# westlake-repl/PixelRec

Hardware: AMD Instinct MI355X
Metric: user-sequences/sec at emb=512 seq_len=50 (SASRec IDNet training step: fwd+bwd+AdamW) (higher is better)
Workload: dtype f32; 1 GPU; BASELINE.json configs[1]: SASRec IDNet emb=512 seq_len=50, 400001 items, 4 heads, inner 2x, 2 layers, BPR loss vs 1 sampled negative, dropout 0.1, AdamW lr 1e-4 wd 0.1; batch_per_gpu=64, global_batch=64, seq_len=50, n_items=400001, embedding_size=512, parallelism=dp1, hip_graph=True

## Files before the change

### include/pxr.h

```cpp
#ifndef PXR_H_
#define PXR_H_
#include <stdint.h>

#ifdef __cplusplus
extern "C" {
#endif

#define PXR_OK 0
#define PXR_ERR_BAD_ARG (-1)
#define PXR_ERR_LAUNCH (-2)
#define PXR_ERR_WORKSPACE (-3)

#define PXR_ABI_VERSION 302
int pxr_version(void);
const char* pxr_last_error(void);
const char* pxr_target_arch(void);

int pxr_dropout_keep_host(uint64_t seed, uint32_t stream_id, uint64_t first_index, int64_t n, float p,
                          uint8_t* keep_out);

int pxr_set_status_word(int32_t* dev_word);

int pxr_embed_gather_f32(const float* table, int64_t N, int D, const int64_t* idx, int64_t n, float* out,
                         void* stream);
// ... 101 lines not shown
                          const int* dy_exp, const int* const* dy_exp_dev, const void* const* x, const int64_t* x_plane_stride,
                          const int64_t* x_panel_rows, const int* x_exp, const int* const* x_exp_dev, float* const* dW,
                          float* const* db, const int* T, const int* N, const int* K, int tile_hint, void* stream);
int pxr_h2_split_auto_multi_f32(int n, const float* const* x, const int64_t* rows, const int64_t* cols, const int64_t* ldx,
                                void* const* planes, const int64_t* plane_stride, const int64_t* panel_rows, int col_stats,
                                float* stats, int* exps, void* stream);
int pxr_h2_bound_exp(const float* a_max, const float* b_colsum, float factor, int* exp_out, void* stream);
int pxr_ln_bwd_stat_f32(const float* dy, const float* xhat, const float* rstd, const float* gamma, int rows, int D, float* dz,
                        float* dx, float* dgamma, float* dbeta, float p_drop, uint64_t seed, uint32_t stream_id,
                        const int64_t* step_dev, void* ws, int64_t ws_bytes, float* stat, float* zero, int zero_n, void* stream);
int pxr_ln_bwd_res_f32(const float* dy, const float* xhat, const float* rstd, const float* gamma, const float* res, int rows, int D,
                       float* dz, float* dgamma, float* dbeta, void* ws, int64_t ws_bytes, float* stat, void* stream);
int pxr_h2_split_parts_f32(const float* x, int64_t rows, int64_t cols, int64_t ldx, void* planes, int64_t plane_stride,
                           int64_t panel_rows, const float* parts, int n_parts, float* stats, int* exps,
                           const float* bound_b_colsum, float bound_factor, int* bound_exp_out, void* stream);
int pxr_attn_bwd_stat_f32(const float* dctx, int64_t ld_ctx, const float* q, const float* k, const float* v, int64_t ld,
                          const float* probs, int B, int H, int L, int d, float* dq, float* dk, float* dv, int64_t ld_d,
                          float p_drop, uint64_t seed, uint32_t stream_id, const int64_t* step_dev, float* stat, void* stream);
int pxr_ln_bwd_h2s_f32(const float* pos_score, const float* neg_score, const float* table, int64_t n_table, const int64_t* items,
                       const int64_t* masked_index, int B, int L, float grad_scale, const float* grad_scale_dev, float* coef,
                       const float* dy, const float* xhat, const float* rstd, const float* gamma, int rows, int D, float* dz,
                       float* dgamma, float* dbeta, float p_drop, uint64_t seed, uint32_t stream_id, const int64_t* step_dev,
                       void* ws, int64_t ws_bytes, void* g_planes, int64_t g_plane_stride, int64_t g_panel_rows,
                       const int* g_exp_dev, float* stat, float* zero, int zero_n, int64_t id_bstride, int64_t pos_off,
                       int64_t neg_off, void* stream);
int pxr_attn_bwd_h2s_f32(const float* dctx, int64_t ld_ctx, const float* q, const float* k, const float* v, int64_t ld,
                         const float* probs, int B, int H, int L, int d, float p_drop, uint64_t seed, uint32_t stream_id,
                         const int64_t* step_dev, void* g_planes, int64_t g_plane_stride, int64_t g_panel_rows, int g_cols,
                         int col_q, int col_k, int col_v, const int* g_exp_dev, float* stat, void* stream);
int pxr_h2_sites_update(int n, const float* const* parts, const int* n_parts, const int* rows, const float* const* bound_b,
                        float bound_factor, int headroom, float decay, float* run_max, int* exps, float* stats, int* bexp, void* stream);

int pxr_attn_planes_supported(int L, int d);
int pxr_score_topk_clock_out(uint64_t* clk2);
int pxr_gemm_reset_flags(void);
int pxr_grouped_dw_planes_f32(int n, const void* const* dy, const int64_t* dy_plane_stride, const int64_t* dy_panel_rows,
                              const void* const* x, const int64_t* x_plane_stride, const int64_t* x_panel_rows,
                              float* const* dW, float* const* db, const int* T, const int* N, const int* K, int tile_hint,
                              void* stream);

int pxr_tower_attn_supported(int T, int d);
int pxr_tower_attn_fwd_f32(const float* q, const float* k, const float* v, int64_t ld, int64_t images, int heads, int T, int d,
                           float scale, float* ctx, int64_t ld_ctx, void* ctx_planes, int64_t ctx_plane_stride,
                           int64_t ctx_panel_rows, int planes_fmt, float* lse, void* stream);
int pxr_tower_attn_bwd_f32(const float* q, const float* k, const float* v, int64_t ld, const float* dctx, const float* ctx,
                           int64_t ld_c, const float* lse, int64_t images, int heads, int T, int d, float scale, float* dq,
                           float* dk, float* dv, int64_t ld_d, float* delta_ws, void* stream);
int pxr_softmax_rows_f32(float* S, int64_t rows, int T, int ld, float scale, void* stream);
int pxr_softmax_rows_bwd_f32(const float* P, float* dP, int64_t rows, int T, int ld, float scale, void* stream);
int pxr_vit_embed_f32(const float* patches, const float* cls, const float* pos, float* out, int64_t n, int T, int H,
                      void* stream);
int pxr_token_mean_f32(const float* x, float* out, int64_t n, int T, int D, void* stream);
int pxr_token_mean_relu_bwd_f32(const float* dout, const float* act, float* dact, int64_t n, int T, int D, void* stream);
int pxr_attn_rows_fwd_f32(float* S, float* PD, const int64_t* keymask, int64_t km_bstride, int B, int H, int L, int ld,
                          float p_drop, uint64_t seed, uint32_t stream_id, const int64_t* step_dev, int d, int causal,
                          void* stream);
int pxr_attn_rows_bwd_f32(const float* P, float* dPD, int B, int H, int L, int ld, float p_drop, uint64_t seed,
                          uint32_t stream_id, const int64_t* step_dev, int d, void* stream);
int pxr_add_f32(const float* a, const float* b, float* out, int64_t n, void* stream);
int pxr_dropout_f32(const float* x, float* y, int64_t n, float p, uint64_t seed, uint32_t stream_id, const int64_t* step_dev,
                    void* stream);

int pxr_linear_fwd_f32(const float* x, const float* W, const float* b, float* y, float* pre, int M, int N, int K,
                       int act, void* stream);
int pxr_linear_bwd_input_f32(const float* dy, const float* W, float* dx, const float* dgelu_pre, const float* add,
                             const float* mul, int M, int N, int K, void* stream);
// ... 240 lines not shown
```

### pixelrec_amd/csrc/attention.hip

```cpp
#include <stdlib.h>

#include "planes.cuh"

namespace pxr {

constexpr int ATT_MAXL = 64;
constexpr int ATT_DC = 128;
constexpr int ATT_KLD = ATT_DC + 4;

#define PXR_ATTN_STAT_SLOTS 64
struct AttnArgs {
  const float* q; const float* k; const float* v;
  int64_t ld;
  const int64_t* keymask; int64_t km_bstride;
  float* ctx; int64_t ld_ctx;
  float* probs;
  const float* dctx; float* dq; float* dk; float* dv; int64_t ld_d;
  int B, H, L, d;
  float sqrt_d;
  float p_drop; uint32_t drop_thr; uint32_t stream; uint64_t seed;
  const int64_t* step_dev;
  P3Mat op;
  int pcol[3];
  int op_fmt;
  int32_t* status;
  const int* gexp;
  float* stat;
};

__device__ __forceinline__ void stage_tile(float* tile, int tstride, const float* src, int64_t ld, int L, int w) {
  const int q4 = w >> 2;
  for (int f = threadIdx.x; f < L * q4; f += blockDim.x) {
    const int row = f / q4, c = (f - row * q4) * 4;
    *reinterpret_cast<float4*>(tile + row * tstride + c) = *reinterpret_cast<const float4*>(src + (int64_t)row * ld + c);
  }
}

template <int NW>
__device__ __forceinline__ void score_accumulate(float (&acc)[64 / NW], const float* sA, const float* sB, int L, int w,
                                                 int wave, int lane) {
  const float* brow = sB + lane * ATT_KLD;
#pragma unroll
  for (int gg = 0; gg < 16 / NW; ++gg) {
    const int i0 = wave + 4 * NW * gg;
    if (i0 >= L) break;
    float a0 = 0.f, a1 = 0.f, a2 = 0.f, a3 = 0.f;
    const float* r0 = sA + (i0)*ATT_DC;
    const float* r1 = sA + (i0 + NW) * ATT_DC;
    const float* r2 = sA + (i0 + 2 * NW) * ATT_DC;
    const float* r3 = sA + (i0 + 3 * NW) * ATT_DC;
    for (int c = 0; c < w; c += 4) {
      const float4 kb = *reinterpret_cast<const float4*>(brow + c);
      const float4 q0 = *reinterpret_cast<const float4*>(r0 + c);
      const float4 q1 = *reinterpret_cast<const float4*>(r1 + c);
      const float4 q2 = *reinterpret_cast<const float4*>(r2 + c);
      const float4 q3 = *reinterpret_cast<const float4*>(r3 + c);
      a0 += q0.x * kb.x + q0.y * kb.y + q0.z * kb.z + q0.w * kb.w;
      a1 += q1.x * kb.x + q1.y * kb.y + q1.z * kb.z + q1.w * kb.w;
      a2 += q2.x * kb.x + q2.y * kb.y + q2.z * kb.z + q2.w * kb.w;
      a3 += q3.x * kb.x + q3.y * kb.y + q3.z * kb.z + q3.w * kb.w;
// ... 579 lines not shown
    const int i = wave + NW * g;
    if (i < L) sS[i * ATT_SLD + lane] = dsrow[g];
  }
  __syncthreads();
  zero_acc<TN>(acc);
  if (mine) lds_mma<true, false, TN>(acc, sS, ATT_SLD, sK, ATT_KLD, wm * 32, n_base, 64, lane);
  if (a.stat && mine) take();
  if (a.dq) store_acc<TN>(acc, a.dq + dbase, a.ld_d, wm * 32, n_base, L, d, lane);
  if (a.op.p) store_acc_planes<TN, NT>(acc, mine, sV, wm * 32, n_base, L, d, lane, a.op, (int64_t)b * L, a.pcol[0] + h * d, PXR_PLANES_BF16X3, a.status, gsc);
  zero_acc<TN>(acc);
  if (mine) lds_mma<false, false, TN>(acc, sS, ATT_SLD, sQ, ATT_KLD, wm * 32, n_base, 64, lane);
  if (a.stat && mine) take();
  if (a.dk) store_acc<TN>(acc, a.dk + dbase, a.ld_d, wm * 32, n_base, L, d, lane);
  if (a.op.p) store_acc_planes<TN, NT>(acc, mine, sV, wm * 32, n_base, L, d, lane, a.op, (int64_t)b * L, a.pcol[1] + h * d, PXR_PLANES_BF16X3, a.status, gsc);
  if (a.stat) {
    __shared__ float smax[NW];
    gmax = wave_max(gmax);
    if (lane == 0) smax[wave] = gmax;
    __syncthreads();
    if (threadIdx.x == 0) {
      float m = smax[0];
#pragma unroll
      for (int w = 1; w < NW; ++w) m = fmaxf(m, smax[w]);
      float* slot = a.stat + (bh & (PXR_ATTN_STAT_SLOTS - 1));
      if (m > __hip_atomic_load(slot, __ATOMIC_RELAXED, __HIP_MEMORY_SCOPE_AGENT)) atomicMax(reinterpret_cast<int*>(slot), __float_as_int(m));
    }
  }
}

constexpr int ATT2_TR = 52;
constexpr int ATT2_NT = 512;
constexpr int ATT2_NP = (ATT2_TR * (ATT_DC / 4) + ATT2_NT - 1) / ATT2_NT;

__device__ __forceinline__ void tile2_load(float4 (&v)[ATT2_NP], const float* src, int64_t ld, int L, int w) {
  const int q4 = w >> 2;
#pragma unroll
  for (int p = 0; p < ATT2_NP; ++p) {
    const int f = threadIdx.x + p * ATT2_NT;
    const int row = f / q4, c = (f - row * q4) * 4;
    v[p] = make_float4(0.f, 0.f, 0.f, 0.f);
    if (row < L) v[p] = *reinterpret_cast<const float4*>(src + (int64_t)row * ld + c);
  }
}
__device__ __forceinline__ void tile2_store(float* tile, const float4 (&v)[ATT2_NP], int L, int w) {
  const int q4 = w >> 2;
#pragma unroll
  for (int p = 0; p < ATT2_NP; ++p) {
    const int f = threadIdx.x + p * ATT2_NT;
    const int row = f / q4, c = (f - row * q4) * 4;
    if (row <= L) *reinterpret_cast<float4*>(tile + row * ATT_KLD + c) = v[p];
  }
}

template <bool A_KC, bool B_KC, int TN>
__device__ __forceinline__ void lds_mma_z(f32x16 (&acc)[TN], const float* sA, int lda, int za, const float* sB, int ldb, int zb,
                                          int m_base, int n_base, int K, int lane) {
  const int h = lane >> 5, r = lane & 31;
  const int arow = min(m_base + r, za);
  int brow[TN];
#pragma unroll
  for (int j = 0; j < TN; ++j) brow[j] = min(n_base + j * 32 + r, zb);
  for (int k0 = 0; k0 < K; k0 += 8) {
    float a[4], b[TN][4];
    if constexpr (A_KC) {
      const float4 v = *reinterpret_cast<const float4*>(sA + arow * lda + k0 + h * 4);
      a[0] = v.x; a[1] = v.y; a[2] = v.z; a[3] = v.w;
    } else {
#pragma unroll
      for (int t = 0; t < 4; ++t) a[t] = sA[min(k0 + h * 4 + t, za) * lda + m_base + r];
    }
#pragma unroll
    for (int j = 0; j < TN; ++j) {
      if constexpr (B_KC) {
        const float4 v = *reinterpret_cast<const float4*>(sB + brow[j] * ldb + k0 + h * 4);
        b[j][0] = v.x; b[j][1] = v.y; b[j][2] = v.z; b[j][3] = v.w;
      } else {
#pragma unroll
        for (int t = 0; t < 4; ++t) b[j][t] = sB[min(k0 + h * 4 + t, zb) * ldb + n_base + j * 32 + r];
      }
    }
#pragma unroll
    for (int t = 0; t < 4; ++t)
#pragma unroll
      for (int j = 0; j < TN; ++j) acc[j] = __builtin_amdgcn_mfma_f32_32x32x2f32(a[t], b[j][t], acc[j], 0, 0, 0);
  }
}

__device__ __forceinline__ void acc_to_tile2(const f32x16& acc, bool mine, float* tile, int m_base, int n_base, int L, int lane) {
  if (!mine) return;
  const int h = lane >> 5, r = lane & 31;
#pragma unroll
  for (int e = 0; e < 16; ++e) {
    const int row = m_base + (e & 3) + 8 * (e >> 2) + 4 * h;
    if (row < L) tile[row * ATT_KLD + n_base + r] = acc[e];
  }
}
__device__ __forceinline__ void tile2_to_planes(const float* tile, int L, int w, const P3Mat& P, int64_t row0, int col0, int fmt,
                                                int32_t* status, float stale_scale = 0.f) {
  const int cpr = w >> 3;
  for (int q = threadIdx.x; q < L * cpr; q += ATT2_NT) {
    const int row = q / cpr, c8 = (q - row * cpr) * 8;
    const float4 x0 = *reinterpret_cast<const float4*>(tile + row * ATT_KLD + c8);
    const float4 x1 = *reinterpret_cast<const float4*>(tile + row * ATT_KLD + c8 + 4);
    const float v[8] = {x0.x, x0.y, x0.z, x0.w, x1.x, x1.y, x1.z, x1.w};
    if (stale_scale != 0.f) px_store8_h2s(P, status, row0 + row, col0 + c8, v, stale_scale);
    else px_store8(P, fmt, status, row0 + row, col0 + c8, v);
  }
}

template <bool CAUSAL>
__device__ __forceinline__ void attn_fwd_mfma2_body(AttnArgs a) {
  if (a.step_dev) a.seed += (uint64_t)a.step_dev[0];
  constexpr int NW = 8;
  __shared__ __attribute__((aligned(16))) float T0[ATT2_TR * ATT_KLD];
  __shared__ __attribute__((aligned(16))) float T1[ATT2_TR * ATT_KLD];
  __shared__ __attribute__((aligned(16))) float sS[ATT_MAXL * ATT_SLD];
  const int lane = threadIdx.x & 63, wave = threadIdx.x >> 6;
  const int bh = xcd_remap(blockIdx.x, gridDim.x), b = bh / a.H, h = bh - b * a.H;
  const int L = a.L, d = a.d, Kp = (L + 7) & ~7;
  const int64_t base = (int64_t)b * L * a.ld + (int64_t)h * d;
  float4 rq[ATT2_NP], rk[ATT2_NP], rv[ATT2_NP];
  tile2_load(rq, a.q + base, a.ld, L, d);
  tile2_load(rk, a.k + base, a.ld, L, d);
  tile2_load(rv, a.v + base, a.ld, L, d);
  const bool key_real = (lane < L) && (a.keymask[(int64_t)b * a.km_bstride + lane] != 0);
  tile2_store(T0, rq, L, d);
  tile2_store(T1, rk, L, d);
  __syncthreads();
  if (wave < 4) {
    const int wm = wave >> 1, wn = wave & 1;
    f32x16 accS[1];
    zero_acc<1>(accS);
    lds_mma_z<true, true, 1>(accS, T0, ATT_KLD, L, T1, ATT_KLD, L, wm * 32, wn * 32, d, lane);
    const int hh = lane >> 5, r = lane & 31;
// ... 119 lines not shown
  __syncthreads();
#pragma unroll
  for (int g = 0; g < ROWS; ++g) {
    const int i = wave + NW * g;
    if (i < L) sS[i * ATT_SLD + lane] = dsrow[g];
  }
  if (a.op.p) {
    acc_to_tile2(acc[0], mine, T0, wm * 32, n_base, L, lane);
    __syncthreads();
    tile2_to_planes(T0, L, d, a.op, (int64_t)b * L, a.pcol[2] + h * d, PXR_PLANES_BF16X3, a.status, gsc);
    __syncthreads();
  }
  tile2_store(T0, r0, L, d);
  __syncthreads();
  zero_acc<1>(acc);
  zero_acc<1>(acc2);
  if (mine) {
    lds_mma_z<true, false, 1>(acc, sS, ATT_SLD, 63, T1, ATT_KLD, L, wm * 32, n_base, Kp, lane);
    lds_mma_z<false, false, 1>(acc2, sS, ATT_SLD, 63, T0, ATT_KLD, L, wm * 32, n_base, Kp, lane);
  }
  if (a.stat && mine) { take(acc[0]); take(acc2[0]); }
  if (a.dq) store_acc<1>(acc, a.dq + dbase, a.ld_d, wm * 32, n_base, L, d, lane);
  if (a.dk) store_acc<1>(acc2, a.dk + dbase, a.ld_d, wm * 32, n_base, L, d, lane);
  if (a.op.p) {
    __syncthreads();
    acc_to_tile2(acc[0], mine, T1, wm * 32, n_base, L, lane);
    acc_to_tile2(acc2[0], mine, T0, wm * 32, n_base, L, lane);
    __syncthreads();
    tile2_to_planes(T1, L, d, a.op, (int64_t)b * L, a.pcol[0] + h * d, PXR_PLANES_BF16X3, a.status, gsc);
    tile2_to_planes(T0, L, d, a.op, (int64_t)b * L, a.pcol[1] + h * d, PXR_PLANES_BF16X3, a.status, gsc);
  }
  if (a.stat) {
    __shared__ float smax[NW];
    gmax = wave_max(gmax);
    if (lane == 0) smax[wave] = gmax;
    __syncthreads();
    if (threadIdx.x == 0) {
      float m = smax[0];
#pragma unroll
      for (int w = 1; w < NW; ++w) m = fmaxf(m, smax[w]);
      float* slot = a.stat + (bh & (PXR_ATTN_STAT_SLOTS - 1));
      if (m > __hip_atomic_load(slot, __ATOMIC_RELAXED, __HIP_MEMORY_SCOPE_AGENT)) atomicMax(reinterpret_cast<int*>(slot), __float_as_int(m));
    }
  }
}

constexpr int ATTL_MAXL = 128;
constexpr int ATTL_SLD = ATTL_MAXL + 4;
constexpr int ATTL_DC = 64;
constexpr int ATTL_KLD = ATTL_DC + 4;
constexpr int ATTL_NT = 512;

__device__ __forceinline__ void stage_tile_long(float* tile, int tstride, const float* src, int64_t ld, int L, int w) {
  const int q4 = w >> 2;
  const int total = ATTL_MAXL * q4;
  float4 v[4];
#pragma unroll
  for (int p = 0; p < 4; ++p) {
    const int f = threadIdx.x + p * ATTL_NT;
    v[p] = make_float4(0.f, 0.f, 0.f, 0.f);
    if (f < total) {
      const int row = f / q4, c = (f - row * q4) * 4;
      if (row < L) v[p] = *reinterpret_cast<const float4*>(src + (int64_t)row * ld + c);
    }
  }
#pragma unroll
// ... 182 lines not shown
}

using namespace pxr;

static int attn_mfma_waves() {
  static const int nw = getenv("PXR_ATTN_MFMA_WAVES") ? atoi(getenv("PXR_ATTN_MFMA_WAVES")) : 8;
  return nw == 8 ? 8 : 4;
}

static int attn_waves() {
  static int nw = 0;
  if (nw == 0) {
    const char* e = getenv("PXR_ATTN_WAVES");
    const int v = e ? atoi(e) : 8;
    nw = (v == 4 || v == 16) ? v : 8;
  }
  return nw;
}

static bool attn_use_two(int L, int d) {
  const char* e = getenv("PXR_ATTN_TWO");
  return L < ATT2_TR && d <= ATT_DC && attn_mfma_waves() == 8 && !(e && atoi(e) == 0);
}

static bool attn_use_mfma(int d) {
  static int flag = -1;
  if (flag < 0) {
    const char* e = getenv("PXR_ATTN_MFMA");
    flag = (e && atoi(e) == 0) ? 0 : 1;
  }
  return flag == 1 && (d % 8) == 0;
}

static int attn_check(int B, int H, int L, int d, int64_t ld, const char* who) {
  PXR_REQUIRE(B >= 0 && H > 0 && L > 0 && d > 0, "%s: bad shape", who);
  PXR_REQUIRE(L <= ATTL_MAXL, "%s: L=%d > %d positions is not supported", who, L, ATTL_MAXL);
  PXR_REQUIRE(L <= ATT_MAXL || (attn_use_mfma(d)), "%s: L=%d > %d needs the MFMA kernels (head size %d %% 8 == 0)", who, L,
              ATT_MAXL, d);
  PXR_REQUIRE(d % 4 == 0 && ld % 4 == 0, "%s: d and ld must be multiples of 4", who);
  return PXR_OK;
}

extern "C" int pxr_attn_planes_supported(int L, int d) { return (L <= ATT_MAXL && attn_use_mfma(d) && d <= ATT_DC && d % 8 == 0) ? 1 : 0; }

extern "C" int pxr_attn_fwd_f32(const float* q, const float* k, const float* v, int64_t ld, const int64_t* keymask,
                                int64_t km_bstride, int B, int H, int L, int d, float* ctx, int64_t ld_ctx, float* probs,
                                float p_drop, uint64_t seed, uint32_t stream_id, const int64_t* step_dev, void* ctx_planes,
                                int64_t ctx_plane_stride, int64_t ctx_panel_rows, int planes_fmt, int causal, void* stream) {
  PXR_REQUIRE(planes_fmt == 0 || planes_fmt == 1, "pxr_attn_fwd_f32: planes_fmt must be 0 (bf16x3) or 1 (h2)");
  PXR_REQUIRE(causal == 0 || causal == 1, "pxr_attn_fwd_f32: causal must be 0 or 1");
  PXR_REQUIRE(planes_fmt == 0 || ctx_planes, "pxr_attn_fwd_f32: h2 output needs planes");
  PXR_REQUIRE(q && k && v && keymask && (ctx || ctx_planes), "pxr_attn_fwd_f32: null pointer");
  PXR_REQUIRE(!ctx_planes || (pxr_attn_planes_supported(L, d) && p3_mat_ok(ctx_planes, ctx_plane_stride, ctx_panel_rows, (int64_t)B * L, (int64_t)H * d)),
              "pxr_attn_fwd_f32: planes are not available for this shape (L=%d, d=%d)", L, d);
  int rc = attn_check(B, H, L, d, ld, "pxr_attn_fwd_f32");
  if (rc) return rc;
  PXR_REQUIRE(p_drop >= 0.f && p_drop < 1.f, "pxr_attn_fwd_f32: bad dropout p");
  if (B == 0) return PXR_OK;
  AttnArgs a{};
  a.q = q; a.k = k; a.v = v; a.ld = ld; a.keymask = keymask; a.km_bstride = km_bstride;
  a.ctx = ctx; a.ld_ctx = ld_ctx; a.probs = probs; a.B = B; a.H = H; a.L = L; a.d = d;
  a.op = P3Mat{reinterpret_cast<__bf16*>(ctx_planes), ctx_plane_stride, ctx_panel_rows};
  a.op_fmt = planes_fmt == 1 ? PXR_PLANES_H2 : PXR_PLANES_BF16X3;
  a.status = pxr_status_word();
  a.sqrt_d = sqrtf((float)d);
  a.p_drop = p_drop; a.drop_thr = pxr_drop_threshold(p_drop); a.stream = stream_id; a.seed = seed;
  a.step_dev = step_dev;
  if (L > ATT_MAXL) {
    hipLaunchKernelGGL(causal ? attn_fwd_long_kernel : attn_fwd_long_bidir_kernel, dim3(B * H), dim3(ATTL_NT), 0, (hipStream_t)stream, a);
    return pxr_check_launch("pxr_attn_fwd_f32(long)");
  }
  if (attn_use_mfma(d)) {
    if (d <= ATT_DC) {
      if (attn_use_two(L, d)) hipLaunchKernelGGL(causal ? attn_fwd_mfma2_kernel : attn_fwd_mfma2_bidir_kernel, dim3(B * H), dim3(ATT2_NT), 0, (hipStream_t)stream, a);
      else if (attn_mfma_waves() == 8) hipLaunchKernelGGL(causal ? attn_fwd_mfma1_kernel<8> : attn_fwd_mfma1_bidir_kernel<8>, dim3(B * H), dim3(512), 0, (hipStream_t)stream, a);
      else hipLaunchKernelGGL(causal ? attn_fwd_mfma1_kernel<4> : attn_fwd_mfma1_bidir_kernel<4>, dim3(B * H), dim3(256), 0, (hipStream_t)stream, a);
    }
    else hipLaunchKernelGGL(causal ? attn_fwd_mfma_kernel : attn_fwd_mfma_bidir_kernel, dim3(B * H), dim3(256), 0, (hipStream_t)stream, a);
    return pxr_check_launch("pxr_attn_fwd_f32(mfma)");
  }
  switch (attn_waves()) {
    case 4: hipLaunchKernelGGL(causal ? attn_fwd_kernel<4> : attn_fwd_bidir_kernel<4>, dim3(B * H), dim3(256), 0, (hipStream_t)stream, a); break;
    case 16: hipLaunchKernelGGL(causal ? attn_fwd_kernel<16> : attn_fwd_bidir_kernel<16>, dim3(B * H), dim3(1024), 0, (hipStream_t)stream, a); break;
    default: hipLaunchKernelGGL(causal ? attn_fwd_kernel<8> : attn_fwd_bidir_kernel<8>, dim3(B * H), dim3(512), 0, (hipStream_t)stream, a); break;
  }
  return pxr_check_launch("pxr_attn_fwd_f32");
}

static int attn_bwd_impl(const float* dctx, int64_t ld_ctx, const float* q, const float* k, const float* v, int64_t ld,
                         const float* probs, int B, int H, int L, int d, float* dq, float* dk, float* dv, int64_t ld_d, float p_drop,
                         uint64_t seed, uint32_t stream_id, const int64_t* step_dev, void* g_planes, int64_t g_plane_stride,
                         int64_t g_panel_rows, int g_cols, int col_q, int col_k, int col_v, float* stat, void* stream,
                         const int* g_exp = nullptr);
extern "C" int pxr_attn_bwd_f32(const float* dctx, int64_t ld_ctx, const float* q, const float* k, const float* v,
                                int64_t ld, const float* probs, int B, int H, int L, int d, float* dq, float* dk,
                                float* dv, int64_t ld_d, float p_drop, uint64_t seed, uint32_t stream_id,
                                const int64_t* step_dev, void* g_planes, int64_t g_plane_stride, int64_t g_panel_rows,
                                int g_cols, int col_q, int col_k, int col_v, void* stream) {
  return attn_bwd_impl(dctx, ld_ctx, q, k, v, ld, probs, B, H, L, d, dq, dk, dv, ld_d, p_drop, seed, stream_id, step_dev, g_planes,
                       g_plane_stride, g_panel_rows, g_cols, col_q, col_k, col_v, nullptr, stream);
}
extern "C" int pxr_attn_bwd_stat_f32(const float* dctx, int64_t ld_ctx, const float* q, const float* k, const float* v, int64_t ld,
                                     const float* probs, int B, int H, int L, int d, float* dq, float* dk, float* dv, int64_t ld_d,
                                     float p_drop, uint64_t seed, uint32_t stream_id, const int64_t* step_dev, float* stat,
                                     void* stream) {
  PXR_REQUIRE(stat && pxr_attn_planes_supported(L, d), "pxr_attn_bwd_stat_f32: no slot, or a shape the fused kernel does not serve (L=%d, d=%d)", L, d);
  return attn_bwd_impl(dctx, ld_ctx, q, k, v, ld, probs, B, H, L, d, dq, dk, dv, ld_d, p_drop, seed, stream_id, step_dev, nullptr, 0, 0, 0,
// ... 8 lines not shown
  return attn_bwd_impl(dctx, ld_ctx, q, k, v, ld, probs, B, H, L, d, nullptr, nullptr, nullptr, 4, p_drop, seed, stream_id, step_dev, g_planes,
                       g_plane_stride, g_panel_rows, g_cols, col_q, col_k, col_v, stat, stream, g_exp_dev);
}
static int attn_bwd_impl(const float* dctx, int64_t ld_ctx, const float* q, const float* k, const float* v, int64_t ld,
                         const float* probs, int B, int H, int L, int d, float* dq, float* dk, float* dv, int64_t ld_d, float p_drop,
                         uint64_t seed, uint32_t stream_id, const int64_t* step_dev, void* g_planes, int64_t g_plane_stride,
                         int64_t g_panel_rows, int g_cols, int col_q, int col_k, int col_v, float* stat, void* stream, const int* g_exp) {
  PXR_REQUIRE(dctx && q && k && v && probs && ((dq && dk && dv) || (g_planes && !dq && !dk && !dv)), "pxr_attn_bwd_f32: null pointer");
  PXR_REQUIRE(!g_exp || (g_planes && stat), "pxr_attn_bwd_h2s_f32: the stale-scale form needs planes and the statistics slots");
  PXR_REQUIRE(!g_planes || (pxr_attn_planes_supported(L, d) && p3_mat_ok(g_planes, g_plane_stride, g_panel_rows, (int64_t)B * L, g_cols) &&
                            col_q % 8 == 0 && col_k % 8 == 0 && col_v % 8 == 0 && col_q >= 0 && col_k >= 0 && col_v >= 0 &&
                            (int64_t)H * d + (col_q > col_k ? (col_q > col_v ? col_q : col_v) : (col_k > col_v ? col_k : col_v)) <= g_cols),
              "pxr_attn_bwd_f32: planes are not available for this shape (L=%d, d=%d) or bad column ranges", L, d);
  int rc = attn_check(B, H, L, d, ld, "pxr_attn_bwd_f32");
  if (rc) return rc;
  PXR_REQUIRE(ld_d % 4 == 0 && ld_ctx % 4 == 0, "pxr_attn_bwd_f32: strides must be multiples of 4");
  if (B == 0) return PXR_OK;
  AttnArgs a{};
  a.q = q; a.k = k; a.v = v; a.ld = ld; a.ld_ctx = ld_ctx; a.probs = const_cast<float*>(probs);
  a.dctx = dctx; a.dq = dq; a.dk = dk; a.dv = dv; a.ld_d = ld_d; a.B = B; a.H = H; a.L = L; a.d = d;
  a.op = P3Mat{reinterpret_cast<__bf16*>(g_planes), g_plane_stride, g_panel_rows};
  a.pcol[0] = col_q; a.pcol[1] = col_k; a.pcol[2] = col_v;
  a.stat = stat;
  a.gexp = g_exp; a.status = pxr_status_word();
  a.sqrt_d = sqrtf((float)d);
  a.p_drop = p_drop; a.drop_thr = pxr_drop_threshold(p_drop); a.stream = stream_id; a.seed = seed;
  a.step_dev = step_dev;
  if (L > ATT_MAXL) {
    hipLaunchKernelGGL(attn_bwd_long_kernel, dim3(B * H), dim3(ATTL_NT), 0, (hipStream_t)stream, a);
    return pxr_check_launch("pxr_attn_bwd_f32(long)");
  }
  if (attn_use_mfma(d)) {
    if (d <= ATT_DC) {
      if (attn_use_two(L, d)) hipLaunchKernelGGL(attn_bwd_mfma2_kernel, dim3(B * H), dim3(ATT2_NT), 0, (hipStream_t)stream, a);
      else if (attn_mfma_waves() == 8) hipLaunchKernelGGL(attn_bwd_mfma1_kernel<8>, dim3(B * H), dim3(512), 0, (hipStream_t)stream, a);
      else hipLaunchKernelGGL(attn_bwd_mfma1_kernel<4>, dim3(B * H), dim3(256), 0, (hipStream_t)stream, a);
    }
    else hipLaunchKernelGGL(attn_bwd_mfma_kernel, dim3(B * H), dim3(256), 0, (hipStream_t)stream, a);
    return pxr_check_launch("pxr_attn_bwd_f32(mfma)");
  }
  switch (attn_waves()) {
    case 4: hipLaunchKernelGGL(attn_bwd_kernel<4>, dim3(B * H), dim3(256), 0, (hipStream_t)stream, a); break;
    case 16: hipLaunchKernelGGL(attn_bwd_kernel<16>, dim3(B * H), dim3(1024), 0, (hipStream_t)stream, a); break;
    default: hipLaunchKernelGGL(attn_bwd_kernel<8>, dim3(B * H), dim3(512), 0, (hipStream_t)stream, a); break;
  }
  return pxr_check_launch("pxr_attn_bwd_f32");
}
```

### pixelrec_amd/lib.py

```python
from __future__ import annotations

import ctypes
import os
from ctypes import c_char_p, c_double, c_float, c_int, c_int64, c_uint64, c_void_p

_HERE = os.path.dirname(os.path.abspath(__file__))
LIB_PATH = os.path.join(_HERE, "libpxr.so")


class PxrError(RuntimeError):
    pass


_lib = None

_P = c_void_p
_F, _D, _I, _I64, _U64, _U32 = c_float, c_double, c_int, c_int64, c_uint64, ctypes.c_uint32
_SIGNATURES = {
    "pxr_version": (c_int, []),
    "pxr_last_error": (c_char_p, []),
    "pxr_target_arch": (c_char_p, []),
    "pxr_dropout_keep_host": (_I, [_U64, _U32, _U64, _I64, _F, _P]),
    "pxr_embed_gather_f32": (_I, [_P, _I64, _I, _P, _I64, _P, _P]),
    "pxr_embed_grad_ws_bytes": (_I64, [_I64]),
# ... 70 lines not shown
    "pxr_causal_im2col_f32": (_I, [_P, _P, _I64, _I, _I, _I, _I, _P]),
    "pxr_causal_col2im_f32": (_I, [_P, _P, _I64, _I, _I, _I, _I, _P]),
    "pxr_gru_gates_fwd_f32": (_I, [_P, _P, _P, _P, _P, _I64, _I, _P]),
    "pxr_gru_gates_bwd_f32": (_I, [_P, _P, _P, _P, _P, _P, _I64, _I, _P]),
    "pxr_softmax_rows_f32": (_I, [_P, _I64, _I, _I, _F, _P]),
    "pxr_softmax_rows_bwd_f32": (_I, [_P, _P, _I64, _I, _I, _F, _P]),
    "pxr_vit_embed_f32": (_I, [_P, _P, _P, _P, _I64, _I, _I, _P]),
    "pxr_token_mean_f32": (_I, [_P, _P, _I64, _I, _I, _P]),
    "pxr_token_mean_relu_bwd_f32": (_I, [_P, _P, _P, _I64, _I, _I, _P]),
    "pxr_add_f32": (_I, [_P, _P, _P, _I64, _P]),
    "pxr_dropout_f32": (_I, [_P, _P, _I64, _F, _U64, _U32, _P, _P]),
    "pxr_attn_rows_fwd_f32": (_I, [_P, _P, _P, _I64, _I, _I, _I, _I, _F, _U64, _U32, _P, _I, _I, _P]),
    "pxr_attn_rows_bwd_f32": (_I, [_P, _P, _I, _I, _I, _I, _F, _U64, _U32, _P, _I, _P]),
    "pxr_split_planes_f32": (_I, [_P, _I64, _I64, _I64, _P, _I64, _I64, _P]),
    "pxr_gemm_planes_f32": (_I, [_I, _I, _I, _I, _P, _I64, _I64, _P, _I64, _I64, _P, _I64, _I, _P, _P, _I64, _P, _I64, _I64,
                                 _I, _I, _P]),
    "pxr_split_planes_multi_f32": (_I, [_I, _P, _P, _P, _P, _P, _P, _P, _P]),
    "pxr_split_h2_multi_f32": (_I, [_I, _P, _P, _P, _P, _P, _P, _P, _P, _P]),
    "pxr_gemm_h2_f32": (_I, [_I, _I, _I, _I, _P, _I64, _I64, _I, _P, _P, _I64, _I64, _I, _P, _P, _I64, _I, _P, _P, _I64, _P, _I64, _I64,
                             _I, _P, _I, _I, _P]),
    "pxr_grouped_dw_h2_f32": (_I, [_I, _P, _P, _P, _P, _P, _P, _P, _P, _P, _P, _P, _P, _P, _P, _P, _I, _P]),
    "pxr_h2_split_auto_multi_f32": (_I, [_I, _P, _P, _P, _P, _P, _P, _P, _I, _P, _P, _P]),
    "pxr_h2_bound_exp": (_I, [_P, _P, _F, _P, _P]),
    "pxr_ln_bwd_stat_f32": (_I, [_P, _P, _P, _P, _I, _I, _P, _P, _P, _P, _F, _U64, _U32, _P, _P, _I64, _P, _P, _I, _P]),
    "pxr_ln_bwd_res_f32": (_I, [_P, _P, _P, _P, _P, _I, _I, _P, _P, _P, _P, _I64, _P, _P]),
    "pxr_h2_split_parts_f32": (_I, [_P, _I64, _I64, _I64, _P, _I64, _I64, _P, _I, _P, _P, _P, _F, _P, _P]),
    "pxr_ln_bwd_h2s_f32": (_I, [_P, _P, _P, _I64, _P, _P, _I, _I, _F, _P, _P, _P, _P, _P, _P, _I, _I, _P, _P, _P, _F, _U64, _U32, _P, _P,
                                _I64, _P, _I64, _I64, _P, _P, _P, _I, _I64, _I64, _I64, _P]),
    "pxr_attn_bwd_h2s_f32": (_I, [_P, _I64, _P, _P, _P, _I64, _P, _I, _I, _I, _I, _F, _U64, _U32, _P, _P, _I64, _I64, _I, _I, _I, _I, _P,
                                  _P, _P]),
    "pxr_h2_sites_update": (_I, [_I, _P, _P, _P, _P, _F, _I, _F, _P, _P, _P, _P, _P]),
    "pxr_attn_bwd_stat_f32": (_I, [_P, _I64, _P, _P, _P, _I64, _P, _I, _I, _I, _I, _P, _P, _P, _I64, _F, _U64, _U32, _P, _P, _P]),
    "pxr_attn_planes_supported": (_I, [_I, _I]),
    "pxr_grouped_dw_planes_f32": (_I, [_I, _P, _P, _P, _P, _P, _P, _P, _P, _P, _P, _P, _I, _P]),
    "pxr_merge_split_rows_f32": (_I, [_P, _P, _I, _I64, _I64, _I, _I64, _F, _P, _P, _P, _P, _I64, _P]),
    "pxr_lgcn_spmm_ws_bytes": (_I64, [_I64, _I]),
    "pxr_lgcn_spmm_f32": (_I, [_P, _P, _P, _I64, _I, _P, _P, _I, _P, _I, _I, _P, _P, _P, _P, _F, _P, _I64, _P]),
    "pxr_lgcn_pair_fwd_f32": (_I, [_P, _I64, _I64, _I, _P, _P, _I, _P, _P, _P, _P, _P, _P]),
    "pxr_lgcn_pair_bwd_f32": (_I, [_P, _I64, _I, _P, _P, _I, _F, _P, _P, _P]),
    "pxr_srgnn_graph_i64": (_I, [_P, _I64, _I, _I64, _P, _P, _P, _P, _P, _P, _P]),
    "pxr_srgnn_prop_f32": (_I, [_P, _I, _I, _I, _P, _P, _P, _I, _P]),
    "pxr_srgnn_readout_fwd_f32": (_I, [_P, _P, _P, _P, _P, _I, _I, _I, _P, _P, _P, _P]),
    "pxr_srgnn_readout_bwd_f32": (_I, [_P, _P, _P, _P, _P, _P, _P, _I, _I, _I, _P, _P, _P, _P]),
    "pxr_srgnn_pair_fwd_f32": (_I, [_P, _I64, _P, _I64, _I, _P, _I, _P, _P, _P, _P]),
    "pxr_srgnn_pair_bwd_f32": (_I, [_P, _I64, _I, _P, _P, _I, _F, _P, _P, _I64, _P, _I64, _P]),
    "pxr_lightsans_fwd_f32": (_I, [_P, _P, _P, _I, _I, _I, _I, _I, _F, _U64, _U32, _P, _P, _P, _P, _P, _P]),
    "pxr_lightsans_bwd_f32": (_I, [_P, _P, _P, _P, _P, _P, _P, _I, _I, _I, _I, _I, _F, _U64, _U32, _P, _P, _P, _P, _P, _P]),
    "pxr_lightsans_pos_fwd_f32": (_I, [_P, _I, _I, _I, _P, _P]),
    "pxr_lightsans_pos_bwd_f32": (_I, [_P, _P, _P, _I, _I, _I, _P, _P]),
    "pxr_table_rows_i64": (_I, [_P, _I, _P, _P, _P]),
    "pxr_mf_pair_fwd_f32": (_I, [_P, _P, _P, _I, _I, _P, _P, _P, _P]),
    "pxr_mf_pair_bwd_f32": (_I, [_P, _P, _P, _I, _I, _F, _P, _P, _P, _P]),
    "pxr_mf_table_grad_f32": (_I, [_P, _I64, _I, _P, _I, _P, _P, _F, _P, _P, _P, _P, _I64, _P]),
    "pxr_mf_bn_tanh_fwd_f32": (_I, [_P, _I, _I, _P, _P, _F, _F, _P, _P, _P, _P, _P, _P, _P]),
    "pxr_mf_bn_tanh_bwd_f32": (_I, [_P, _P, _P, _P, _P, _P, _I, _I, _P, _P, _P, _P]),
    "pxr_mf_bn_tanh_eval_f32": (_I, [_P, _I64, _I, _P, _P, _P, _P, _F, _P, _P]),
    "pxr_vbpr_gather_f32": (_I, [_P, _I64, _I, _P, _I64, _P, _P, _P, _P]),
    "pxr_vbpr_pair_fwd_f32": (_I, [_P, _P, _P, _P, _I, _I, _P, _P, _P, _P]),
    "pxr_vbpr_pair_bwd_f32": (_I, [_P, _P, _P, _P, _I, _I, _F, _P, _P, _P, _P, _P, _P, _I64, _P]),
    "pxr_vbpr_bias_grad_f32": (_I, [_P, _P, _I, _I, _P, _P]),
    "pxr_vbpr_pack_f32": (_I, [_P, _P, _P, _P, _P, _I64, _I, _I, _P, _P]),
    "pxr_curator_pool_f32": (_I, [_P, _P, _I64, _I, _I, _I, _P, _P, _P]),
    "pxr_curator_pool_bwd_f32": (_I, [_P, _P, _P, _P, _I, _I, _I, _P, _P]),
    "pxr_mul_f32": (_I, [_P, _P, _P, _I64, _P]),
    "pxr_curator_pair_fwd_f32": (_I, [_P, _P, _I, _I, _P, _P, _P, _P]),
    "pxr_acf_region_fwd_f32": (_I, [_P, _P, _P, _P, _P, _I, _I, _I, _I, _P, _P, _P]),
# ... 99 lines not shown
```

### pixelrec_amd/ops.py

```python
from __future__ import annotations

import ctypes
import os

import torch

from . import lib as _l

_CHECK_IDX = os.environ.get("PXR_CHECK_INDICES", "0") == "1"


def _req(t: torch.Tensor, dtype, name: str, contiguous: bool = True):
    if not isinstance(t, torch.Tensor) or not t.is_cuda:
        raise _l.PxrError(f"{name}: expected a CUDA/HIP tensor (pixelrec_amd has no CPU fallback)")
    if t.dtype != dtype:
        raise _l.PxrError(f"{name}: expected dtype {dtype}, got {t.dtype}")
    if contiguous and not t.is_contiguous():
        raise _l.PxrError(f"{name}: expected a contiguous tensor")
    return t


class Workspace:

    def __init__(self):
# ... 1046 lines not shown
    Lb = _l.load()
    D, ld, Lp, bh = H * d, 3 * H * d, (L + 3) & ~3, B * H
    P = torch.empty(bh, L, Lp, dtype=torch.float32, device=qkv.device)
    sP, sQ, sC = (H * L * Lp, L * Lp), (L * ld, d), (L * D, d)
    gemm_batched(True, True, L, L, d, qkv, 0, ld, qkv, D, ld, P, 0, Lp, bh, H, sQ, sQ, sP)
    PD = torch.empty_like(P) if p_drop > 0 else None
    _l.check(Lb.pxr_attn_rows_fwd_f32(_l.ptr(P), _l.ptr(PD), _l.ptr(keymask), km_bstride, B, H, L, Lp, p_drop, seed, stream_id,
                                      _l.ptr(step_dev), d, int(causal), _l.stream_ptr()), "pxr_attn_rows_fwd_f32")
    ctx = torch.empty(B, L, D, dtype=torch.float32, device=qkv.device)
    gemm_batched(True, False, L, d, L, PD if PD is not None else P, 0, Lp, qkv, 2 * D, ld, ctx, 0, D, bh, H, sP, sQ, sC)
    return ctx, (P, PD)


def _attn_long_bwd(dctx, qkv, saved, B, H, L, d, p_drop, seed, stream_id, step_dev):
    Lb = _l.load()
    P, PD = saved
    D, ld, Lp, bh = H * d, 3 * H * d, (L + 3) & ~3, B * H
    sP, sQ, sC = (H * L * Lp, L * Lp), (L * ld, d), (L * D, d)
    dqkv = torch.empty_like(qkv)
    gemm_batched(False, False, L, d, L, PD if PD is not None else P, 0, Lp, dctx, 0, D, dqkv, 2 * D, ld, bh, H, sP, sC, sQ)
    dP = torch.empty_like(P)
    gemm_batched(True, True, L, L, d, dctx, 0, D, qkv, 2 * D, ld, dP, 0, Lp, bh, H, sC, sQ, sP)
    _l.check(Lb.pxr_attn_rows_bwd_f32(_l.ptr(P), _l.ptr(dP), B, H, L, Lp, p_drop, seed, stream_id, _l.ptr(step_dev), d,
                                      _l.stream_ptr()), "pxr_attn_rows_bwd_f32")
    gemm_batched(True, False, L, d, L, dP, 0, Lp, qkv, D, ld, dqkv, 0, ld, bh, H, sP, sQ, sQ)
    gemm_batched(False, False, L, d, L, dP, 0, Lp, qkv, 0, ld, dqkv, D, ld, bh, H, sP, sQ, sQ)
    return dqkv


def attn_planes_supported(L: int, d: int) -> bool:
    return bool(_l.load().pxr_attn_planes_supported(L, d))


def attn_fwd(qkv, keymask, km_bstride, B, H, L, d, p_drop=0.0, seed=0, stream_id=0, save=True, step_dev=None,
             planes: bool = False, causal: bool = True):
    Lb = _l.load()
    _req(qkv, torch.float32, "qkv"); _req(keymask, torch.int64, "keymask", contiguous=False)
    D = H * d
    if _attn_takes_gemm_path(L, d):
        ctx, saved = _attn_long_fwd(qkv, keymask, km_bstride, B, H, L, d, p_drop, seed, stream_id, step_dev, causal=causal)
        return (split_planes(ctx.view(B * L, D)) if planes else ctx), (saved if save else None)
    fused_p = planes and attn_planes_supported(L, d)
    h2 = planes == "h2"
    assert fused_p or not h2, "h2 context planes come from the fused kernel only (attn_planes_supported)"
    ctx = None if fused_p else torch.empty(B, L, D, dtype=torch.float32, device=qkv.device)
    cp_ = Planes.alloc(B * L, D, qkv.device, fmt=int(h2)) if fused_p else None
    probs = torch.empty(B, H, L, L, dtype=torch.float32, device=qkv.device) if save else None
    base = qkv.data_ptr()
    q, k, v = _l.c_void_p(base), _l.c_void_p(base + 4 * D), _l.c_void_p(base + 8 * D)
    _l.check(Lb.pxr_attn_fwd_f32(q, k, v, 3 * D, _l.ptr(keymask), km_bstride, B, H, L, d, _l.ptr(ctx), D, _l.ptr(probs), p_drop, seed,
                                 stream_id, _l.ptr(step_dev), *_pl(cp_), int(h2), int(causal), _l.stream_ptr()), "pxr_attn_fwd_f32")
    if planes and not fused_p:
        cp_ = split_planes(ctx.view(B * L, D))
    return (cp_ if planes else ctx), probs


def attn_bwd(dctx, qkv, probs, B, H, L, d, p_drop=0.0, seed=0, stream_id=0, step_dev=None, planes: bool = False,
             stat: torch.Tensor | None = None):
    Lb = _l.load()
    D = H * d
    if stat is not None:
        assert not planes and attn_planes_supported(L, d) and stat.numel() >= ATTN_STAT_SLOTS
        _req(dctx, torch.float32, "dctx"); _req(qkv, torch.float32, "qkv"); _req(probs, torch.float32, "probs")
        dqkv = torch.empty_like(qkv)
        cp = _l.c_void_p
        base, g = qkv.data_ptr(), dqkv.data_ptr()
# ... 1513 lines not shown
```

Measured before the change: 92490 sequences/s.

## Split attention backward across two blocks per head to fill idle CUs

Adds split-attention kernels that launch two blocks per (batch, head). In forward the two blocks split the query rows; in backward one block computes dV while the other computes dQ and dK. Blocks are ordered with an XCD-aware remap. Backward uses the split by default when B*H does not exceed the CU count (64*4=256 here); forward split stays off by default. This trades some duplicated loads of K, V, dctx and probs for twice as many blocks, so more of the GPU is busy when B*H alone underfills it.

```diff
diff --git a/include/pxr.h b/include/pxr.h
--- a/include/pxr.h
+++ b/include/pxr.h
@@ -157,6 +157,7 @@
                         float bound_factor, int headroom, float decay, float* run_max, int* exps, float* stats, int* bexp, void* stream);
 
 int pxr_attn_planes_supported(int L, int d);
+int pxr_attn_split_used(int B, int H, int L, int d, int backward);
 int pxr_score_topk_clock_out(uint64_t* clk2);
 int pxr_gemm_reset_flags(void);
 int pxr_grouped_dw_planes_f32(int n, const void* const* dy, const int64_t* dy_plane_stride, const int64_t* dy_panel_rows,
diff --git a/pixelrec_amd/csrc/attention.hip b/pixelrec_amd/csrc/attention.hip
--- a/pixelrec_amd/csrc/attention.hip
+++ b/pixelrec_amd/csrc/attention.hip
@@ -26,6 +26,7 @@
   int32_t* status;
   const int* gexp;
   float* stat;
+  int split_order;
 };
 
 __device__ __forceinline__ void stage_tile(float* tile, int tstride, const float* src, int64_t ld, int L, int w) {
@@ -671,23 +672,23 @@
 constexpr int ATT2_NT = 512;
 constexpr int ATT2_NP = (ATT2_TR * (ATT_DC / 4) + ATT2_NT - 1) / ATT2_NT;
 
-__device__ __forceinline__ void tile2_load(float4 (&v)[ATT2_NP], const float* src, int64_t ld, int L, int w) {
+__device__ __forceinline__ void tile2_load(float4 (&v)[ATT2_NP], const float* src, int64_t ld, int L, int w, int lo = 0, int hi = ATT2_TR) {
   const int q4 = w >> 2;
 #pragma unroll
   for (int p = 0; p < ATT2_NP; ++p) {
     const int f = threadIdx.x + p * ATT2_NT;
     const int row = f / q4, c = (f - row * q4) * 4;
     v[p] = make_float4(0.f, 0.f, 0.f, 0.f);
-    if (row < L) v[p] = *reinterpret_cast<const float4*>(src + (int64_t)row * ld + c);
-  }
-}
-__device__ __forceinline__ void tile2_store(float* tile, const float4 (&v)[ATT2_NP], int L, int w) {
+    if (row < L && row >= lo && row < hi) v[p] = *reinterpret_cast<const float4*>(src + (int64_t)row * ld + c);
+  }
+}
+__device__ __forceinline__ void tile2_store(float* tile, const float4 (&v)[ATT2_NP], int L, int w, int lo = 0, int hi = ATT2_TR) {
   const int q4 = w >> 2;
 #pragma unroll
   for (int p = 0; p < ATT2_NP; ++p) {
     const int f = threadIdx.x + p * ATT2_NT;
     const int row = f / q4, c = (f - row * q4) * 4;
-    if (row <= L) *reinterpret_cast<float4*>(tile + row * ATT_KLD + c) = v[p];
+    if (row <= L && ((row >= lo && row < hi) || row == L)) *reinterpret_cast<float4*>(tile + row * ATT_KLD + c) = v[p];
   }
 }
 
@@ -735,10 +736,10 @@
   }
 }
 __device__ __forceinline__ void tile2_to_planes(const float* tile, int L, int w, const P3Mat& P, int64_t row0, int col0, int fmt,
-                                                int32_t* status, float stale_scale = 0.f) {
+                                                int32_t* status, float stale_scale = 0.f, int lo = 0) {
   const int cpr = w >> 3;
-  for (int q = threadIdx.x; q < L * cpr; q += ATT2_NT) {
-    const int row = q / cpr, c8 = (q - row * cpr) * 8;
+  for (int q = threadIdx.x; q < (L - lo) * cpr; q += ATT2_NT) {
+    const int row = lo + q / cpr, c8 = (q - (row - lo) * cpr) * 8;
     const float4 x0 = *reinterpret_cast<const float4*>(tile + row * ATT_KLD + c8);
     const float4 x1 = *reinterpret_cast<const float4*>(tile + row * ATT_KLD + c8 + 4);
     const float v[8] = {x0.x, x0.y, x0.z, x0.w, x1.x, x1.y, x1.z, x1.w};
@@ -924,6 +925,213 @@
   }
   if (a.stat) {
     __shared__ float smax[NW];
+    gmax = wave_max(gmax);
+    if (lane == 0) smax[wave] = gmax;
+    __syncthreads();
+    if (threadIdx.x == 0) {
+      float m = smax[0];
+#pragma unroll
+      for (int w = 1; w < NW; ++w) m = fmaxf(m, smax[w]);
+      float* slot = a.stat + (bh & (PXR_ATTN_STAT_SLOTS - 1));
+      if (m > __hip_atomic_load(slot, __ATOMIC_RELAXED, __HIP_MEMORY_SCOPE_AGENT)) atomicMax(reinterpret_cast<int*>(slot), __float_as_int(m));
+    }
+  }
+}
+
+__device__ __forceinline__ int split_block(const AttnArgs& a, int& which) {
+  const int n = gridDim.x >> 1;
+  if (a.split_order == 0) { which = blockIdx.x & 1; return blockIdx.x >> 1; }
+  which = (int)blockIdx.x >= n;
+  return xcd_remap(blockIdx.x - which * n, n);
+}
+
+template <bool CAUSAL>
+__device__ __forceinline__ void attn_fwd_split_body(AttnArgs a) {
+  if (a.step_dev) a.seed += (uint64_t)a.step_dev[0];
+  constexpr int NW = 8;
+  __shared__ __attribute__((aligned(16))) float T0[ATT2_TR * ATT_KLD];
+  __shared__ __attribute__((aligned(16))) float T1[ATT2_TR * ATT_KLD];
+  __shared__ __attribute__((aligned(16))) float sS[ATT_MAXL * ATT_SLD];
+  const int lane = threadIdx.x & 63, wave = threadIdx.x >> 6;
+  int half;
+  const int bh = split_block(a, half), b = bh / a.H, h = bh - b * a.H;
+  const int L = a.L, d = a.d, Kp = (L + 7) & ~7;
+  const int lo = half * 32, hi = min(lo + 32, L);
+  const int64_t base = (int64_t)b * L * a.ld + (int64_t)h * d;
+  float4 rq[ATT2_NP], rk[ATT2_NP], rv[ATT2_NP];
+  tile2_load(rq, a.q + base, a.ld, L, d, lo, hi);
+  tile2_load(rk, a.k + base, a.ld, L, d);
+  tile2_load(rv, a.v + base, a.ld, L, d);
+  const bool key_real = (lane < L) && (a.keymask[(int64_t)b * a.km_bstride + lane] != 0);
+  tile2_store(T0, rq, L, d, lo, hi);
+  tile2_store(T1, rk, L, d);
+  __syncthreads();
+  if ((wave >> 1) == half) {
+    const int wn = wave & 1;
+    f32x16 accS[1];
+    zero_acc<1>(accS);
+    lds_mma_z<true, true, 1>(accS, T0, ATT_KLD, L, T1, ATT_KLD, L, lo, wn * 32, d, lane);
+    const int hh = lane >> 5, r = lane & 31;
+#pragma unroll
+    for (int e = 0; e < 16; ++e)
+      sS[(lo + (e & 3) + 8 * (e >> 2) + 4 * hh) * ATT_SLD + wn * 32 + r] = accS[0][e];
+  }
+  __syncthreads();
+  tile2_store(T0, rv, L, d);
+  const bool drop = a.drop_thr != 0u;
+  const float inv_keep = 1.0f / (1.0f - a.p_drop);
+  for (int i = lo + wave; i < hi; i += NW) {
+    float s = sS[i * ATT_SLD + lane] / a.sqrt_d + ((key_real && (!CAUSAL || lane <= i)) ? 0.0f : -1e9f);
+    if (lane >= L) s = -INFINITY;
+    const float m = wave_max(s);
+    const float e = (lane < L) ? expf(s - m) : 0.f;
+    const float sum = wave_sum(e);
+    const float p = e / sum;
+    float pd = 0.f;
+    if (lane < L) {
+      const int64_t pi = (((int64_t)b * a.H + h) * L + i) * L + lane;
+      if (a.probs) a.probs[pi] = p;
+      pd = p;
+      if (drop) pd = pxr_keep(a.seed, a.stream, (uint64_t)pi, a.drop_thr) ? p * inv_keep : 0.f;
+    }
+    sS[i * ATT_SLD + lane] = pd;
+  }
+  __syncthreads();
+  float* ctx = a.ctx + (int64_t)b * L * a.ld_ctx + (int64_t)h * d;
+  const int n_base = (wave & 3) * 32;
+  const bool mine = wave < 4 && n_base < d;
+  f32x16 accO[1];
+  zero_acc<1>(accO);
+  if (mine) lds_mma_z<true, false, 1>(accO, sS, ATT_SLD, 63, T0, ATT_KLD, L, lo, n_base, Kp, lane);
+  if (a.ctx && mine) store_acc<1>(accO, ctx, a.ld_ctx, lo, n_base, L, d, lane);
+  if (a.op.p) {
+    acc_to_tile2(accO[0], mine, T1, lo, n_base, L, lane);
+    __syncthreads();
+    tile2_to_planes(T1, hi, d, a.op, (int64_t)b * L, h * d, a.op_fmt, a.status, 0.f, lo);
+  }
+}
+__global__ void __launch_bounds__(ATT2_NT, 4) attn_fwd_split_kernel(AttnArgs a) { attn_fwd_split_body<true>(a); }
+__global__ void __launch_bounds__(ATT2_NT, 4) attn_fwd_split_bidir_kernel(AttnArgs a) { attn_fwd_split_body<false>(a); }
+
+__global__ void __launch_bounds__(ATT2_NT, 4) attn_bwd_split_kernel(AttnArgs a) {
+  if (a.step_dev) a.seed += (uint64_t)a.step_dev[0];
+  constexpr int NW = 8, ROWS = 64 / NW;
+  __shared__ __attribute__((aligned(16))) float T0[ATT2_TR * ATT_KLD];
+  __shared__ __attribute__((aligned(16))) float T1[ATT2_TR * ATT_KLD];
+  __shared__ __attribute__((aligned(16))) float sS[ATT_MAXL * ATT_SLD];
+  __shared__ float smax[NW];
+  const int lane = threadIdx.x & 63, wave = threadIdx.x >> 6;
+  int role_v;
+  const int bh = split_block(a, role_v), b = bh / a.H, h = bh - b * a.H;
+  const int L = a.L, d = a.d, Kp = (L + 7) & ~7;
+  const int64_t base = (int64_t)b * L * a.ld + (int64_t)h * d;
+  const int64_t cbase = (int64_t)b * L * a.ld_ctx + (int64_t)h * d;
+  const int64_t dbase = (int64_t)b * L * a.ld_d + (int64_t)h * d;
+  float4 r0[ATT2_NP], r1[ATT2_NP];
+  tile2_load(r0, a.dctx + cbase, a.ld_ctx, L, d);
+  if (!role_v) tile2_load(r1, a.v + base, a.ld, L, d);
+  float prow[ROWS];
+#pragma unroll
+  for (int g = 0; g < ROWS; ++g) {
+    const int i = wave + NW * g;
+    prow[g] = (i < L && lane < L) ? a.probs[(((int64_t)b * a.H + h) * L + i) * L + lane] : 0.f;
+  }
+  const bool drop = a.drop_thr != 0u;
+  const float inv_keep = 1.0f / (1.0f - a.p_drop);
+  const int wm = wave >> 2, n_base = (wave & 3) * 32;
+  const bool mine = n_base < d;
+  const float gsc = a.gexp ? ldexpf(1.0f, a.gexp[0]) : 0.f;
+  float gmax = 0.f;
+  auto take = [&](const f32x16& acc) {
+    const bool col_ok = n_base + (lane & 31) < d;
+#pragma unroll
+    for (int e = 0; e < 16; ++e) {
+      const int row = wm * 32 + (e & 3) + 8 * (e >> 2) + 4 * (lane >> 5);
+      if (col_ok && row < L) gmax = fmaxf(gmax, fabsf(acc[e]));
+    }
+  };
+  f32x16 acc[1], acc2[1];
+  zero_acc<1>(acc);
+  if (role_v) {
+    tile2_store(T0, r0, L, d);
+#pragma unroll
+    for (int g = 0; g < ROWS; ++g) {
+      const int i = wave + NW * g;
+      if (i < Kp) {
+        float pd = 0.f;
+        if (i < L && lane < L) {
+          const int64_t pi = (((int64_t)b * a.H + h) * L + i) * L + lane;
+          const bool keep = !drop || pxr_keep(a.seed, a.stream, (uint64_t)pi, a.drop_thr);
+          const float kf = drop ? (keep ? inv_keep : 0.f) : 1.f;
+          pd = prow[g] * kf;
+        }
+        sS[i * ATT_SLD + lane] = pd;
+      }
+    }
+    __syncthreads();
+    if (mine) lds_mma_z<false, false, 1>(acc, sS, ATT_SLD, 63, T0, ATT_KLD, L, wm * 32, n_base, Kp, lane);
+    if (a.stat && mine) take(acc[0]);
+    if (a.dv) store_acc<1>(acc, a.dv + dbase, a.ld_d, wm * 32, n_base, L, d, lane);
+    if (a.op.p) {
+      __syncthreads();
+      acc_to_tile2(acc[0], mine, T0, wm * 32, n_base, L, lane);
+      __syncthreads();
+      tile2_to_planes(T0, L, d, a.op, (int64_t)b * L, a.pcol[2] + h * d, PXR_PLANES_BF16X3, a.status, gsc);
+    }
+  } else {
+    tile2_store(T0, r0, L, d);
+    tile2_store(T1, r1, L, d);
+    tile2_load(r1, a.k + base, a.ld, L, d);
+    tile2_load(r0, a.q + base, a.ld, L, d);
+    __syncthreads();
+    if (wave < 4) {
+      const int sm = wave >> 1, sn = wave & 1;
+      f32x16 accP[1];
+      zero_acc<1>(accP);
+      lds_mma_z<true, true, 1>(accP, T0, ATT_KLD, L, T1, ATT_KLD, L, sm * 32, sn * 32, d, lane);
+      const int hh = lane >> 5, r = lane & 31;
+#pragma unroll
+      for (int e = 0; e < 16; ++e)
+        sS[(sm * 32 + (e & 3) + 8 * (e >> 2) + 4 * hh) * ATT_SLD + sn * 32 + r] = accP[0][e];
+    }
+    __syncthreads();
+    tile2_store(T1, r1, L, d);
+    tile2_store(T0, r0, L, d);
+#pragma unroll
+    for (int g = 0; g < ROWS; ++g) {
+      const int i = wave + NW * g;
+      if (i < L) {
+        const float p = prow[g];
+        float dp = 0.f;
+        if (lane < L) {
+          const int64_t pi = (((int64_t)b * a.H + h) * L + i) * L + lane;
+          const bool keep = !drop || pxr_keep(a.seed, a.stream, (uint64_t)pi, a.drop_thr);
+          const float kf = drop ? (keep ? inv_keep : 0.f) : 1.f;
+          dp = sS[i * ATT_SLD + lane] * kf;
+        }
+        const float t = wave_sum(dp * p);
+        sS[i * ATT_SLD + lane] = (lane < L) ? p * (dp - t) / a.sqrt_d : 0.f;
+      }
+    }
+    __syncthreads();
+    zero_acc<1>(acc2);
+    if (mine) {
+      lds_mma_z<true, false, 1>(acc, sS, ATT_SLD, 63, T1, ATT_KLD, L, wm * 32, n_base, Kp, lane);
+      lds_mma_z<false, false, 1>(acc2, sS, ATT_SLD, 63, T0, ATT_KLD, L, wm * 32, n_base, Kp, lane);
+    }
+    if (a.stat && mine) { take(acc[0]); take(acc2[0]); }
+    if (a.dq) store_acc<1>(acc, a.dq + dbase, a.ld_d, wm * 32, n_base, L, d, lane);
+    if (a.dk) store_acc<1>(acc2, a.dk + dbase, a.ld_d, wm * 32, n_base, L, d, lane);
+    if (a.op.p) {
+      __syncthreads();
+      acc_to_tile2(acc[0], mine, T1, wm * 32, n_base, L, lane);
+      acc_to_tile2(acc2[0], mine, T0, wm * 32, n_base, L, lane);
+      __syncthreads();
+      tile2_to_planes(T1, L, d, a.op, (int64_t)b * L, a.pcol[0] + h * d, PXR_PLANES_BF16X3, a.status, gsc);
+      tile2_to_planes(T0, L, d, a.op, (int64_t)b * L, a.pcol[1] + h * d, PXR_PLANES_BF16X3, a.status, gsc);
+    }
+  }
+  if (a.stat) {
     gmax = wave_max(gmax);
     if (lane == 0) smax[wave] = gmax;
     __syncthreads();
@@ -1172,6 +1380,32 @@
   return flag == 1 && (d % 8) == 0;
 }
 
+static int attn_cu_count() {
+  static int cus = -1;
+  if (cus < 0) {
+    int dev = 0, n = 0;
+    if (hipGetDevice(&dev) != hipSuccess || hipDeviceGetAttribute(&n, hipDeviceAttributeMultiprocessorCount, dev) != hipSuccess) {
+      (void)hipGetLastError();
+      n = 0;
+    }
+    cus = n;
+  }
+  return cus;
+}
+
+constexpr bool ATTN_SPLIT_DEFAULT_FWD = false, ATTN_SPLIT_DEFAULT_BWD = true;
+static bool attn_use_split(int B, int H, int L, int d, bool backward) {
+  const char* e = getenv("PXR_ATTN_SPLIT");
+  const int v = e ? atoi(e) : 1;
+  const bool on = e ? (v != 0 && v != (backward ? 2 : 3)) : (backward ? ATTN_SPLIT_DEFAULT_BWD : ATTN_SPLIT_DEFAULT_FWD);
+  if (!on) return false;
+  return attn_use_mfma(d) && attn_use_two(L, d) && (backward || L > 32) && (int64_t)B * H <= attn_cu_count();
+}
+static int attn_split_order() {
+  const char* e = getenv("PXR_ATTN_SPLIT_ORDER");
+  return e ? (atoi(e) != 0) : 1;
+}
+
 static int attn_check(int B, int H, int L, int d, int64_t ld, const char* who) {
   PXR_REQUIRE(B >= 0 && H > 0 && L > 0 && d > 0, "%s: bad shape", who);
   PXR_REQUIRE(L <= ATTL_MAXL, "%s: L=%d > %d positions is not supported", who, L, ATTL_MAXL);
@@ -1182,6 +1416,9 @@
 }
 
 extern "C" int pxr_attn_planes_supported(int L, int d) { return (L <= ATT_MAXL && attn_use_mfma(d) && d <= ATT_DC && d % 8 == 0) ? 1 : 0; }
+extern "C" int pxr_attn_split_used(int B, int H, int L, int d, int backward) {
+  return (B > 0 && H > 0 && L > 0 && d > 0 && attn_use_split(B, H, L, d, backward != 0)) ? 1 : 0;
+}
 
 extern "C" int pxr_attn_fwd_f32(const float* q, const float* k, const float* v, int64_t ld, const int64_t* keymask,
                                 int64_t km_bstride, int B, int H, int L, int d, float* ctx, int64_t ld_ctx, float* probs,
@@ -1212,7 +1449,11 @@
   }
   if (attn_use_mfma(d)) {
     if (d <= ATT_DC) {
-      if (attn_use_two(L, d)) hipLaunchKernelGGL(causal ? attn_fwd_mfma2_kernel : attn_fwd_mfma2_bidir_kernel, dim3(B * H), dim3(ATT2_NT), 0, (hipStream_t)stream, a);
+      if (attn_use_split(B, H, L, d, false)) {
+        a.split_order = attn_split_order();
+        hipLaunchKernelGGL(causal ? attn_fwd_split_kernel : attn_fwd_split_bidir_kernel, dim3(2 * B * H), dim3(ATT2_NT), 0, (hipStream_t)stream, a);
+      }
+      else if (attn_use_two(L, d)) hipLaunchKernelGGL(causal ? attn_fwd_mfma2_kernel : attn_fwd_mfma2_bidir_kernel, dim3(B * H), dim3(ATT2_NT), 0, (hipStream_t)stream, a);
       else if (attn_mfma_waves() == 8) hipLaunchKernelGGL(causal ? attn_fwd_mfma1_kernel<8> : attn_fwd_mfma1_bidir_kernel<8>, dim3(B * H), dim3(512), 0, (hipStream_t)stream, a);
       else hipLaunchKernelGGL(causal ? attn_fwd_mfma1_kernel<4> : attn_fwd_mfma1_bidir_kernel<4>, dim3(B * H), dim3(256), 0, (hipStream_t)stream, a);
     }
@@ -1287,7 +1528,11 @@
   }
   if (attn_use_mfma(d)) {
     if (d <= ATT_DC) {
-      if (attn_use_two(L, d)) hipLaunchKernelGGL(attn_bwd_mfma2_kernel, dim3(B * H), dim3(ATT2_NT), 0, (hipStream_t)stream, a);
+      if (attn_use_split(B, H, L, d, true)) {
+        a.split_order = attn_split_order();
+        hipLaunchKernelGGL(attn_bwd_split_kernel, dim3(2 * B * H), dim3(ATT2_NT), 0, (hipStream_t)stream, a);
+      }
+      else if (attn_use_two(L, d)) hipLaunchKernelGGL(attn_bwd_mfma2_kernel, dim3(B * H), dim3(ATT2_NT), 0, (hipStream_t)stream, a);
       else if (attn_mfma_waves() == 8) hipLaunchKernelGGL(attn_bwd_mfma1_kernel<8>, dim3(B * H), dim3(512), 0, (hipStream_t)stream, a);
       else hipLaunchKernelGGL(attn_bwd_mfma1_kernel<4>, dim3(B * H), dim3(256), 0, (hipStream_t)stream, a);
     }
diff --git a/pixelrec_amd/lib.py b/pixelrec_amd/lib.py
--- a/pixelrec_amd/lib.py
+++ b/pixelrec_amd/lib.py
@@ -126,6 +126,7 @@
     "pxr_h2_sites_update": (_I, [_I, _P, _P, _P, _P, _F, _I, _F, _P, _P, _P, _P, _P]),
     "pxr_attn_bwd_stat_f32": (_I, [_P, _I64, _P, _P, _P, _I64, _P, _I, _I, _I, _I, _P, _P, _P, _I64, _F, _U64, _U32, _P, _P, _P]),
     "pxr_attn_planes_supported": (_I, [_I, _I]),
+    "pxr_attn_split_used": (_I, [_I, _I, _I, _I, _I]),
     "pxr_grouped_dw_planes_f32": (_I, [_I, _P, _P, _P, _P, _P, _P, _P, _P, _P, _P, _P, _I, _P]),
     "pxr_merge_split_rows_f32": (_I, [_P, _P, _I, _I64, _I64, _I, _I64, _F, _P, _P, _P, _P, _I64, _P]),
     "pxr_lgcn_spmm_ws_bytes": (_I64, [_I64, _I]),
diff --git a/pixelrec_amd/ops.py b/pixelrec_amd/ops.py
--- a/pixelrec_amd/ops.py
+++ b/pixelrec_amd/ops.py
@@ -1102,6 +1102,10 @@
     return bool(_l.load().pxr_attn_planes_supported(L, d))
 
 
+def attn_split_used(B: int, H: int, L: int, d: int, backward: bool) -> bool:
+    return bool(_l.load().pxr_attn_split_used(B, H, L, d, int(backward)))
+
+
 def attn_fwd(qkv, keymask, km_bstride, B, H, L, d, p_drop=0.0, seed=0, stream_id=0, save=True, step_dev=None,
              planes: bool = False, causal: bool = True):
     Lb = _l.load()
```

Measured after the change: 92970 sequences/s (median of 6 runs). No clear change (+0.5%).
